# can-lehmann/exprgrad

Hardware: AMD Instinct MI355X
Metric: GFLOP/s matmul 4096^3 f32 (1 GPU) (higher is better)
Workload: dtype f32

## Files before the change

### exprgrad_amd/csrc/kernels/gemm_split_bf16.hip

```cpp
#include <algorithm>
#include <cfloat>

#include "gemm_fused.hpp"
#include "../eg_internal.hpp"
#include "../switches.hpp"

namespace {

typedef __bf16 bf16x8 __attribute__((ext_vector_type(8)));
typedef __bf16 bf16x4 __attribute__((ext_vector_type(4)));
typedef float f32x4 __attribute__((ext_vector_type(4)));


struct SplitOperand {
  const float* src;
  long ld;
  long R;
  int kc;
  __bf16* dst;
};

__device__ __forceinline__ void unit_coords(const SplitOperand& o, long K, long u, long& r, long& chunk) {
  const long cpr = K / 8, t = u >> 6;
  const int l = (int)(u & 63);
  if (o.kc) {
    const long per = cpr / 4;
    r = (t / per) * 16 + (l >> 2);
    chunk = (t % per) * 4 + (l & 3);
  } else {
    const long per = cpr / 2;
    r = (t / per) * 32 + (l >> 1);
    chunk = (t % per) * 2 + (l & 1);
  }
}

__device__ __forceinline__ void load_unit(const SplitOperand& o, long r, long chunk, float (&x)[8]) {
  if (o.kc) {
    const f32x4* p = reinterpret_cast<const f32x4*>(o.src + r * o.ld + chunk * 8);
    const f32x4 v0 = __builtin_nontemporal_load(p), v1 = __builtin_nontemporal_load(p + 1);
#pragma unroll
    for (int j = 0; j < 4; ++j) {
      x[j] = v0[j];
      x[4 + j] = v1[j];
    }
  } else {
    const float* p = o.src + chunk * 8 * o.ld + r;
#pragma unroll
    for (int j = 0; j < 8; ++j) x[j] = __builtin_nontemporal_load(p + j * o.ld);
  }
}

__device__ __forceinline__ void split_elem(float v, __bf16& b0, __bf16& b1, __bf16& b2, bool& bad) {
  b0 = (__bf16)v;
  const float r1 = v - (float)b0;
  b1 = (__bf16)r1;
  const float f1 = (float)b1;
  const float r2 = r1 - f1;
  b2 = (__bf16)r2;
  const float f2 = (float)b2;
  bad |= !(r2 == f2);
  bad |= v != 0.f && __builtin_fabsf(v) < FLT_MIN;
  bad |= (f1 != 0.f && __builtin_fabsf(f1) < FLT_MIN) || (f2 != 0.f && __builtin_fabsf(f2) < FLT_MIN);
}

__device__ __forceinline__ void split_unit(const SplitOperand& o, long K, long r, long chunk, const float (&x)[8], bool& bad) {
  bf16x8 h0, h1, h2;
#pragma unroll
  for (int j = 0; j < 8; ++j) {
    __bf16 b0, b1, b2;
    split_elem(x[j], b0, b1, b2, bad);
    h0[j] = b0;
    h1[j] = b1;
    h2[j] = b2;
  }
  const long plane = o.R * K;
  bf16x8* d = reinterpret_cast<bf16x8*>(o.dst + ((chunk >> 1) * o.R + r) * 16 + (chunk & 1) * 8);
  const long ps = plane / 8;
  d[0] = h0;
  d[ps] = h1;
  d[2 * ps] = h2;
}

constexpr int SPLIT_NT = 256;
constexpr int SPLIT_U = 2;

template <int U>
__device__ __forceinline__ void split_units(const SplitOperand& a, const SplitOperand& b, long K, long units_a, long lo, long hi,
                                            bool& bad) {
  constexpr long STEP = (long)SPLIT_NT * U;
  for (long base = lo; base < hi; base += STEP) {
    float x[U][8];
    long r[U], c[U];
#pragma unroll
    for (int i = 0; i < U; ++i) {
      const long u = base + i * SPLIT_NT + threadIdx.x;
      if (u >= hi) continue;
      const bool in_a = u < units_a;
      unit_coords(in_a ? a : b, K, in_a ? u : u - units_a, r[i], c[i]);
      load_unit(in_a ? a : b, r[i], c[i], x[i]);
    }
#pragma unroll
    for (int i = 0; i < U; ++i) {
      const long u = base + i * SPLIT_NT + threadIdx.x;
      if (u >= hi) continue;
      split_unit(u < units_a ? a : b, K, r[i], c[i], x[i], bad);
    }
  }
}

__global__ __launch_bounds__(SPLIT_NT) void split_planes_kernel(SplitOperand a, SplitOperand b, long K, long units_a, long units,
                                                              unsigned* flag, unsigned epoch) {
  constexpr long STEP = (long)SPLIT_NT * SPLIT_U;
  const long per = ((units + gridDim.x - 1) / gridDim.x + STEP - 1) / STEP * STEP;
  const long lo = (long)blockIdx.x * per, hi = lo + per < units ? lo + per : units;
  bool bad = false;
  split_units<SPLIT_U>(a, b, K, units_a, lo, hi, bad);
  if (__builtin_expect(bad, 0)) *(volatile unsigned*)flag = epoch;
}

constexpr int TILE_R = 256;
constexpr int REC_BYTES = 8 * 32 + 16;
constexpr int IMG_PLANE = (TILE_R / 8) * REC_BYTES;
constexpr int IMG_BYTES = 3 * IMG_PLANE;
constexpr int TILE_BLOCKS_PER_CU = 3;

__device__ __forceinline__ void load_tile(const SplitOperand& o, long kt, long rb, f32x4 (&x)[4]) {
  const int wave = threadIdx.x >> 6, lane = threadIdx.x & 63;
  const float* p = o.src + (kt * 16 + wave * 4) * o.ld + rb * TILE_R + lane * 4;
#pragma unroll
  for (int i = 0; i < 4; ++i) x[i] = __builtin_nontemporal_load(reinterpret_cast<const f32x4*>(p + i * o.ld));
}

__device__ __forceinline__ void split_tile(const f32x4 (&x)[4], unsigned char* img, bool& bad) {
  const int wave = threadIdx.x >> 6, lane = threadIdx.x & 63;
  unsigned char* row = img + (lane >> 1) * REC_BYTES + (lane & 1) * 128 + wave * 8;
#pragma unroll
  for (int c = 0; c < 4; ++c) {
    bf16x4 h0, h1, h2;
#pragma unroll
    for (int i = 0; i < 4; ++i) {
      __bf16 b0, b1, b2;
      split_elem(x[i][c], b0, b1, b2, bad);
      h0[i] = b0;
      h1[i] = b1;
      h2[i] = b2;
    }
    *reinterpret_cast<bf16x4*>(row + c * 32) = h0;
    *reinterpret_cast<bf16x4*>(row + c * 32 + IMG_PLANE) = h1;
    *reinterpret_cast<bf16x4*>(row + c * 32 + 2 * IMG_PLANE) = h2;
  }
}

__device__ __forceinline__ int lane_unit(int lane) {
  const int quad = (lane >> 2) & 7;
  return ((lane >> 5) * 2 + (__builtin_popcount(quad) & 1)) * 16 + (quad >> 1) * 4 + (lane & 3);
}

__device__ __forceinline__ void store_tile(const SplitOperand& o, long K, long kt, long rb, const unsigned char* img) {
  const int wave = threadIdx.x >> 6, lane = threadIdx.x & 63;
  const long plane = o.R * K;
  __bf16* d = o.dst + (kt * o.R + rb * TILE_R) * 16;
#pragma unroll
  for (int p = 0; p < 3; ++p)
#pragma unroll
    for (int i = 0; i < 2; ++i) {
      const int u = (wave * 2 + i) * 64 + lane_unit(lane);
      const bf16x8 v = *reinterpret_cast<const bf16x8*>(img + p * IMG_PLANE + (u >> 4) * REC_BYTES + (u & 15) * 16);
      *reinterpret_cast<bf16x8*>(d + p * plane + u * 8) = v;
    }
}

__global__ __launch_bounds__(SPLIT_NT) void split_tiles_kernel(SplitOperand a, SplitOperand b, long K, int tiled, unsigned* flag,
                                                             unsigned epoch) {
  __shared__ __attribute__((aligned(16))) unsigned char img[2][IMG_BYTES];
  bool bad = false;
  int s = 0;
#pragma unroll
  for (int which = 0; which < 2; ++which) {
    const SplitOperand& o = which ? b : a;
    const long n = o.R * K / (TILE_R * 16);
    const long lo = n * blockIdx.x / gridDim.x, hi = n * (blockIdx.x + 1) / gridDim.x;
    if (!(tiled >> which & 1)) {
      const long units = o.R * K / 8;
      split_units<SPLIT_U>(o, o, K, units, lo * (SPLIT_NT * 2), hi * (SPLIT_NT * 2), bad);
      continue;
    }
    if (lo >= hi) continue;
    const long tr = o.R / TILE_R;
    long kt = lo / tr, rb = lo % tr;
    f32x4 x[4];
    load_tile(o, kt, rb, x);
    for (long t = lo; t < hi; ++t) {
      split_tile(x, img[s], bad);
      long nkt = kt, nrb = rb + 1;
      if (nrb == tr) {
        nrb = 0;
        ++nkt;
      }
      if (t + 1 < hi) load_tile(o, nkt, nrb, x);
      __syncthreads();
      store_tile(o, K, kt, rb, img[s]);
      s ^= 1;
      kt = nkt;
      rb = nrb;
    }
  }
  if (__builtin_expect(bad, 0)) *(volatile unsigned*)flag = epoch;
}


constexpr int BM = 256, BN = 256, WM = 128, WN = 64, NT = 512;
constexpr int STAGES = 3;
constexpr int PLANE_BYTES = BM * 16 * 2;
constexpr int STAGE_BYTES = 6 * PLANE_BYTES;
constexpr int LOADS = STAGE_BYTES / (NT * 16);

struct SplitGemmArgs {
  const __bf16* pa;
  const __bf16* pb;
  float* C;
  const float* bias;
  long M, N, K, ldc;
  int tiles_m, tiles_n;
  int accumulate;
  int skew;
  const unsigned* flag;
  unsigned epoch;
};

__device__ __forceinline__ int xcd_remap(int bid, int nwg) {
  constexpr int NXCD = 8;
  const int q = nwg / NXCD, r = nwg % NXCD;
  const int xcd = bid % NXCD, local = bid / NXCD;
  return (xcd < r ? xcd * (q + 1) : r * (q + 1) + (xcd - r) * q) + local;
}
__device__ __forceinline__ void tile_origin(int wgid, int tiles_m, int tiles_n, long& m_blk, long& n_blk) {
  constexpr int GROUP = 8;
  const int per_group = GROUP * tiles_n;
  const int first_m = (wgid / per_group) * GROUP;
  const int gsize = min(tiles_m - first_m, GROUP);
  const int in_group = wgid % per_group;
  m_blk = (long)(first_m + in_group % gsize) * BM;
  n_blk = (long)(in_group / gsize) * BN;
}

__device__ __forceinline__ const void* uniform_ptr(const void* p) {
  const unsigned long v = reinterpret_cast<unsigned long>(p);
  const unsigned lo = __builtin_amdgcn_readfirstlane((unsigned)v), hi = __builtin_amdgcn_readfirstlane((unsigned)(v >> 32));
  return reinterpret_cast<const void*>(((unsigned long)hi << 32) | lo);
}

constexpr int ROLE_LOAD_OWN = 1, ROLE_LOAD_PARTNER = 2, ROLE_READ_TOP = 4, ROLE_READ_AHEAD = 8;
constexpr int PARTNER = 4;

#ifdef EG_SPLIT_GEMM_STAMPS
constexpr int STAMP_BLOCKS = 1024;
__device__ unsigned long long g_split_stamps[STAMP_BLOCKS][8][4];
#define EG_STAMP(t)                                                                  \
  do {                                                                               \
    __builtin_amdgcn_sched_barrier(0);                                               \
    asm volatile("s_memtime %0\n\ts_waitcnt lgkmcnt(0)" : "=s"(t)::"memory"); \
    __builtin_amdgcn_sched_barrier(0);                                               \
  } while (0)
#else
#define EG_STAMP(t) \
  do {              \
  } while (0)
#endif

__global__ __launch_bounds__(NT) void split_gemm_kernel(SplitGemmArgs a) {
  if (*(volatile const unsigned*)a.flag == a.epoch) return;
  __shared__ __attribute__((aligned(16))) unsigned char lds[STAGES * STAGE_BYTES];

  const int tid = threadIdx.x, lane = tid & 63, wave = __builtin_amdgcn_readfirstlane(tid >> 6);
  const int wr = wave >> 2, wc = wave & 3;
  long m_blk, n_blk;
  tile_origin(xcd_remap(blockIdx.x, gridDim.x), a.tiles_m, a.tiles_n, m_blk, n_blk);

  const __amdgpu_buffer_rsrc_t ra = __builtin_amdgcn_make_buffer_rsrc(
      const_cast<void*>(uniform_ptr(a.pa + m_blk * 16)), (short)0, -1, 0x00020000);
  const __amdgpu_buffer_rsrc_t rb = __builtin_amdgcn_make_buffer_rsrc(
      const_cast<void*>(uniform_ptr(a.pb + n_blk * 16)), (short)0, -1, 0x00020000);
  const unsigned a_plane = (unsigned)(a.M * a.K * 2), b_plane = (unsigned)(a.N * a.K * 2);
  const unsigned a_ktile = (unsigned)(a.M * 32), b_ktile = (unsigned)(a.N * 32);
  const unsigned voff = (unsigned)lane * 16;

  auto pieces = [&](int kt, int s, int w) {
    unsigned char* st = lds + s * STAGE_BYTES + w * 1024;
    const unsigned at = (unsigned)kt * a_ktile + (unsigned)w * 1024, bt = (unsigned)kt * b_ktile + (unsigned)w * 1024;
#pragma unroll
    for (int i = 0; i < LOADS; ++i) {
      __attribute__((address_space(3))) void* dst = (__attribute__((address_space(3))) void*)(st + i * PLANE_BYTES);
      if (i < 3)
        __builtin_amdgcn_raw_ptr_buffer_load_lds(ra, dst, 16, voff, (unsigned)i * a_plane + at, 0, 0);
      else
        __builtin_amdgcn_raw_ptr_buffer_load_lds(rb, dst, 16, voff, (unsigned)(i - 3) * b_plane + bt, 0, 0);
    }
  };
  auto issue = [&](int kt, int s, int r) {
    if (r & ROLE_LOAD_OWN) pieces(kt, s, wave);
    if (r & ROLE_LOAD_PARTNER) pieces(kt, s, wave ^ PARTNER);
  };

  f32x4 acc[8][4];
#pragma unroll
  for (int i = 0; i < 8; ++i)
#pragma unroll
    for (int j = 0; j < 4; ++j)
#pragma unroll
      for (int r = 0; r < 4; ++r) acc[i][j][r] = 0.f;

  const int sel = lane >> 5;
  const int a_row = (wr * WM + (lane & 15)) * 32 + ((lane >> 4) & 1) * 16;
  const int b_row = 3 * PLANE_BYTES + (wc * WN + (lane & 15)) * 32 + ((lane >> 4) & 1) * 16;
  const int a01_off = a_row + sel * PLANE_BYTES, a02_off = a_row + 2 * sel * PLANE_BYTES;
  const int b21_off = b_row + (2 - sel) * PLANE_BYTES, b10_off = b_row + (1 - sel) * PLANE_BYTES, b00_off = b_row;

  bf16x8 fb21[4], fb10[4], fb00[4], fa01, fa02;
  auto read_head = [&](const unsigned char* st) {
#pragma unroll
    for (int j = 0; j < 4; ++j) {
      fb21[j] = *reinterpret_cast<const bf16x8*>(st + b21_off + j * 512);
      fb10[j] = *reinterpret_cast<const bf16x8*>(st + b10_off + j * 512);
      fb00[j] = *reinterpret_cast<const bf16x8*>(st + b00_off + j * 512);
    }
    fa01 = *reinterpret_cast<const bf16x8*>(st + a01_off);
    fa02 = *reinterpret_cast<const bf16x8*>(st + a02_off);
  };
#pragma unroll
  for (int j = 0; j < 4; ++j) fb21[j] = fb10[j] = fb00[j] = bf16x8{};
  fa01 = fa02 = bf16x8{};

  const int skew = a.skew;
  const int role = !skew ? ROLE_LOAD_OWN | ROLE_READ_TOP
                         : (wave & PARTNER) ? ROLE_LOAD_OWN | ROLE_LOAD_PARTNER | ROLE_READ_TOP : ROLE_READ_AHEAD;
  const int KT = (int)(a.K / 16);
  issue(0, 0, role);
  if (KT > 1) issue(1, 1, role);
  if (skew) {
    if (KT > 1) asm volatile("s_waitcnt vmcnt(12)" ::: "memory");
    else asm volatile("s_waitcnt vmcnt(0)" ::: "memory");
    __builtin_amdgcn_s_barrier();
    asm volatile("" ::: "memory");
    if (role & ROLE_READ_AHEAD) read_head(lds);
  }
#ifdef EG_SPLIT_GEMM_STAMPS
  unsigned long long t0 = 0, t1 = 0, t2 = 0, front = 0, body = 0, back = 0;
#endif
  int s = 0;
  for (int kt = 0; kt < KT; ++kt) {
    if (!skew && kt + 1 < KT) asm volatile("s_waitcnt vmcnt(6)" ::: "memory");
    else asm volatile("s_waitcnt vmcnt(0)" ::: "memory");
    __builtin_amdgcn_s_barrier();
    asm volatile("" ::: "memory");
#ifdef EG_SPLIT_GEMM_STAMPS
    EG_STAMP(t0);
    if (kt) back += t0 - t2;
#endif
    int r = role;
    asm volatile("" : "+s"(r));
    if (kt + 2 < KT) issue(kt + 2, s == 0 ? 2 : s - 1, r);
    const unsigned char* st = lds + s * STAGE_BYTES;
    if (r & ROLE_READ_TOP) read_head(st);
    EG_STAMP(t1);
    bf16x8 c01 = fa01, c02 = fa02;
#pragma unroll
    for (int i = 0; i < 8; ++i) {
      bf16x8 n01 = c01, n02 = c02;
      __builtin_amdgcn_sched_barrier(0);
      if (i + 1 < 8) {
        n01 = *reinterpret_cast<const bf16x8*>(st + a01_off + (i + 1) * 512);
        n02 = *reinterpret_cast<const bf16x8*>(st + a02_off + (i + 1) * 512);
      }
      __builtin_amdgcn_sched_barrier(0);
#pragma unroll
      for (int j = 0; j < 4; ++j) acc[i][j] = __builtin_amdgcn_mfma_f32_16x16x32_bf16(c01, fb21[j], acc[i][j], 0, 0, 0);
#pragma unroll
      for (int j = 0; j < 4; ++j) acc[i][j] = __builtin_amdgcn_mfma_f32_16x16x32_bf16(c01, fb10[j], acc[i][j], 0, 0, 0);
#pragma unroll
      for (int j = 0; j < 4; ++j) acc[i][j] = __builtin_amdgcn_mfma_f32_16x16x32_bf16(c02, fb00[j], acc[i][j], 0, 0, 0);
      c01 = n01;
      c02 = n02;
    }
    EG_STAMP(t2);
#ifdef EG_SPLIT_GEMM_STAMPS
    front += t1 - t0;
    body += t2 - t1;
#endif
    s = s == STAGES - 1 ? 0 : s + 1;
    if ((r & ROLE_READ_AHEAD) && kt + 1 < KT) read_head(lds + s * STAGE_BYTES);
  }
#ifdef EG_SPLIT_GEMM_STAMPS
  if (lane == 0 && blockIdx.x < STAMP_BLOCKS) {
    unsigned long long* o = g_split_stamps[blockIdx.x][wave];
    o[0] = front;
    o[1] = body;
    o[2] = back;
    o[3] = (unsigned long long)KT;
  }
#endif

  __syncthreads();
  float* park = reinterpret_cast<float*>(lds) + wave * 64 * WN;
  const int prow = lane >> 4, pc4 = (lane & 15) * 4;
  const long col = n_blk + wc * WN + pc4;
  f32x4 b4 = {0.f, 0.f, 0.f, 0.f};
  if (a.bias) b4 = *reinterpret_cast<const f32x4*>(a.bias + col);
#pragma unroll
  for (int h = 0; h < 2; ++h) {
#pragma unroll
    for (int i = 0; i < 4; ++i)
#pragma unroll
      for (int j = 0; j < 4; ++j)
#pragma unroll
        for (int r = 0; r < 4; ++r) park[(i * 16 + 4 * prow + r) * WN + j * 16 + (lane & 15)] = acc[4 * h + i][j][r];
    asm volatile("s_waitcnt lgkmcnt(0)" ::: "memory");
#pragma unroll
    for (int q = 0; q < 16; ++q) {
      const int row = 4 * q + prow;
      f32x4 v = *reinterpret_cast<const f32x4*>(park + row * WN + pc4);
      f32x4* c = reinterpret_cast<f32x4*>(a.C + (m_blk + wr * WM + h * 64 + row) * a.ldc + col);
      if (a.accumulate) v = *c + v;
      if (a.bias) v = v + b4;
      *c = v;
    }
    asm volatile("s_waitcnt lgkmcnt(0)" ::: "memory");
  }
}

inline bool aligned16(const void* p) { return (reinterpret_cast<uintptr_t>(p) & 15) == 0; }

constexpr size_t kPlaneCap = 1ull << 30;

}

namespace eg {
namespace gemm {

int sgemm_split(eg_ctx* ctx, int trans_a, int trans_b, long M, long N, long K, const float* A, long lda, const float* B, long ldb,
                float* C, long ldc, int accumulate, const float* bias) {
  if (!ctx || !A || !B || !C || M <= 0 || N <= 0 || K <= 0) return EG_ERR_UNSUPPORTED;
  if (lda < (trans_a ? M : K) || ldb < (trans_b ? K : N) || ldc < N) return EG_ERR_UNSUPPORTED;
  if (eg::sw::on(eg::Sw::NO_SPLIT_GEMM)) return EG_ERR_UNSUPPORTED;
  if (M % BM != 0 || N % BN != 0 || K % 32 != 0 || K < 2048) return EG_ERR_UNSUPPORTED;
  if ((M / BM) * (N / BN) < ctx->compute_units) return EG_ERR_UNSUPPORTED;
  const size_t plane_bytes = 6 * (size_t)(M + N) * (size_t)K;
  if (plane_bytes > kPlaneCap || 6 * (size_t)std::max(M, N) * (size_t)K >= (1ull << 31)) return EG_ERR_UNSUPPORTED;
  if (!aligned16(A) || !aligned16(B) || (!trans_a && lda % 4 != 0) || (trans_b && ldb % 4 != 0)) return EG_ERR_UNSUPPORTED;
  if (!aligned16(C) || ldc % 4 != 0 || (bias && !aligned16(bias))) return EG_ERR_UNSUPPORTED;
  if (!exact_single_launch(ctx, trans_a, trans_b, M, N, K, A, lda, B, ldb, C, ldc, bias)) return EG_ERR_UNSUPPORTED;

  int rc = eg::set_device(ctx);
  if (rc) return rc;
  if (!ctx->split_flag) {
    EG_HIP_CHECK(hipMalloc((void**)&ctx->split_flag, sizeof(unsigned)));
    EG_HIP_CHECK(hipMemset(ctx->split_flag, 0, sizeof(unsigned)));
  }
  rc = eg::ensure_workspace(ctx, plane_bytes);
  if (rc) return rc;
  if (++ctx->split_epoch == 0) ctx->split_epoch = 1;
  const unsigned epoch = ctx->split_epoch;

  __bf16* pa = static_cast<__bf16*>(ctx->workspace);
  __bf16* pb = pa + 3 * (size_t)M * K;
  const SplitOperand oa = {A, lda, M, trans_a ? 0 : 1, pa};
  const SplitOperand ob = {B, ldb, N, trans_b ? 1 : 0, pb};
  const bool scalar = eg::sw::on(eg::Sw::SPLIT_PASS_SCALAR);
  const int tiled = (!scalar && !oa.kc && lda % 4 == 0 ? 1 : 0) | (!scalar && !ob.kc && ldb % 4 == 0 ? 2 : 0);
  if (tiled) {
    const long blocks = (long)TILE_BLOCKS_PER_CU * ctx->compute_units;
    hipLaunchKernelGGL(split_tiles_kernel, dim3((unsigned)blocks), dim3(SPLIT_NT), 0, ctx->stream, oa, ob, K, tiled, ctx->split_flag,
                       epoch);
  } else {
    const long units_a = M * K / 8, units = (M + N) * K / 8;
    long blocks = (units + SPLIT_NT * SPLIT_U - 1) / (SPLIT_NT * SPLIT_U);
    if (blocks > 8L * ctx->compute_units) blocks = 8L * ctx->compute_units;
    hipLaunchKernelGGL(split_planes_kernel, dim3((unsigned)blocks), dim3(SPLIT_NT), 0, ctx->stream, oa, ob, K, units_a, units,
                       ctx->split_flag, epoch);
  }
  EG_HIP_CHECK(hipGetLastError());

  SplitGemmArgs g = {};
  g.pa = pa;
  g.pb = pb;
  g.C = C;
  g.bias = bias;
  g.M = M;
  g.N = N;
  g.K = K;
  g.ldc = ldc;
  g.tiles_m = (int)(M / BM);
  g.tiles_n = (int)(N / BN);
  g.accumulate = accumulate;
  g.skew = eg::sw::on(eg::Sw::GEMM_NO_SKEW) ? 0 : 1;
  g.flag = ctx->split_flag;
  g.epoch = epoch;
  hipLaunchKernelGGL(split_gemm_kernel, dim3((unsigned)(g.tiles_m * g.tiles_n)), dim3(NT), 0, ctx->stream, g);
  EG_HIP_CHECK(hipGetLastError());

  return sgemm_exact(ctx, trans_a, trans_b, M, N, K, A, lda, B, ldb, C, ldc, accumulate, bias, ctx->split_flag, epoch);
}

}
}

#ifdef EG_SPLIT_GEMM_STAMPS
extern "C" int eg_debug_split_stamps(unsigned long long* dst, size_t count) {
  if (count > sizeof(g_split_stamps) / sizeof(unsigned long long)) return EG_ERR_UNSUPPORTED;
  EG_HIP_CHECK(hipDeviceSynchronize());
  EG_HIP_CHECK(hipMemcpyFromSymbol(dst, HIP_SYMBOL(g_split_stamps), count * sizeof(unsigned long long)));
  return 0;
}
#endif
```

Baseline: 261,500.

## Add ping-pong split GEMM kernel with producer/consumer wave roles

Adds a templated split_product with a PINGPONG variant. In it, one half of the waves (role Y) issues all global-to-LDS loads for both halves, and the two halves are staggered by one barrier so that their MFMA phases alternate, with s_setprio raising priority during multiply. The default launch now uses the ping-pong kernel, and the old skewed kernel becomes reachable only via the NO_SKEW switch with skew forced to 0. The aim is better overlap of LDS reads, global loads and MFMA across wave groups. The cost is two barriers per k-tile and a more delicate vmcnt schedule.

```diff
diff --git a/exprgrad_amd/csrc/kernels/gemm_split_bf16.hip b/exprgrad_amd/csrc/kernels/gemm_split_bf16.hip
--- a/exprgrad_amd/csrc/kernels/gemm_split_bf16.hip
+++ b/exprgrad_amd/csrc/kernels/gemm_split_bf16.hip
@@ -2,6 +2,7 @@
 #include <cfloat>
 
 #include "gemm_fused.hpp"
+#include "split_schedule.hpp"
 #include "../eg_internal.hpp"
 #include "../switches.hpp"
 
@@ -268,9 +269,40 @@
   } while (0)
 #endif
 
-__global__ __launch_bounds__(NT) void split_gemm_kernel(SplitGemmArgs a) {
+__device__ __forceinline__ void store_c(const SplitGemmArgs& a, unsigned char (&lds)[STAGES * STAGE_BYTES], const f32x4 (&acc)[8][4], long m_blk,
+                                        long n_blk, int wave, int lane) {
+  const int wr = wave >> 2, wc = wave & 3;
+  __syncthreads();
+  float* park = reinterpret_cast<float*>(lds) + wave * 64 * WN;
+  const int prow = lane >> 4, pc4 = (lane & 15) * 4;
+  const long col = n_blk + wc * WN + pc4;
+  f32x4 b4 = {0.f, 0.f, 0.f, 0.f};
+  if (a.bias) b4 = *reinterpret_cast<const f32x4*>(a.bias + col);
+#pragma unroll
+  for (int h = 0; h < 2; ++h) {
+#pragma unroll
+    for (int i = 0; i < 4; ++i)
+#pragma unroll
+      for (int j = 0; j < 4; ++j)
+#pragma unroll
+        for (int r = 0; r < 4; ++r) park[(i * 16 + 4 * prow + r) * WN + j * 16 + (lane & 15)] = acc[4 * h + i][j][r];
+    asm volatile("s_waitcnt lgkmcnt(0)" ::: "memory");
+#pragma unroll
+    for (int q = 0; q < 16; ++q) {
+      const int row = 4 * q + prow;
+      f32x4 v = *reinterpret_cast<const f32x4*>(park + row * WN + pc4);
+      f32x4* c = reinterpret_cast<f32x4*>(a.C + (m_blk + wr * WM + h * 64 + row) * a.ldc + col);
+      if (a.accumulate) v = *c + v;
+      if (a.bias) v = v + b4;
+      *c = v;
+    }
+    asm volatile("s_waitcnt lgkmcnt(0)" ::: "memory");
+  }
+}
+
+template <bool PINGPONG>
+__device__ __forceinline__ void split_product(const SplitGemmArgs& a, unsigned char (&lds)[STAGES * STAGE_BYTES]) {
   if (*(volatile const unsigned*)a.flag == a.epoch) return;
-  __shared__ __attribute__((aligned(16))) unsigned char lds[STAGES * STAGE_BYTES];
 
   const int tid = threadIdx.x, lane = tid & 63, wave = __builtin_amdgcn_readfirstlane(tid >> 6);
   const int wr = wave >> 2, wc = wave & 3;
@@ -330,6 +362,77 @@
 #pragma unroll
   for (int j = 0; j < 4; ++j) fb21[j] = fb10[j] = fb00[j] = bf16x8{};
   fa01 = fa02 = bf16x8{};
+
+  auto multiply = [&](const unsigned char* st) {
+    bf16x8 c01 = fa01, c02 = fa02;
+#pragma unroll
+    for (int i = 0; i < 8; ++i) {
+      bf16x8 n01 = c01, n02 = c02;
+      __builtin_amdgcn_sched_barrier(0);
+      if (i + 1 < 8) {
+        n01 = *reinterpret_cast<const bf16x8*>(st + a01_off + (i + 1) * 512);
+        n02 = *reinterpret_cast<const bf16x8*>(st + a02_off + (i + 1) * 512);
+      }
+      __builtin_amdgcn_sched_barrier(0);
+#pragma unroll
+      for (int j = 0; j < 4; ++j) acc[i][j] = __builtin_amdgcn_mfma_f32_16x16x32_bf16(c01, fb21[j], acc[i][j], 0, 0, 0);
+#pragma unroll
+      for (int j = 0; j < 4; ++j) acc[i][j] = __builtin_amdgcn_mfma_f32_16x16x32_bf16(c01, fb10[j], acc[i][j], 0, 0, 0);
+#pragma unroll
+      for (int j = 0; j < 4; ++j) acc[i][j] = __builtin_amdgcn_mfma_f32_16x16x32_bf16(c02, fb00[j], acc[i][j], 0, 0, 0);
+      c01 = n01;
+      c02 = n02;
+    }
+  };
+
+  if constexpr (PINGPONG) {
+    namespace ss = eg::split_sched;
+    static_assert(ss::STAGES == STAGES && ss::PIECES == 2 * LOADS && ss::WAVES * 64 == NT, "split_schedule.hpp is this kernel's");
+    auto issue_both = [&](int kt, int s) {
+      pieces(kt, s, wave);
+      pieces(kt, s, wave ^ PARTNER);
+    };
+    const int role = ss::role_of(wave);
+    const int KT = (int)(a.K / 16);
+    if (role == ss::Y) {
+      for (int t = 0; t < ss::prologue_tiles(ss::Y, KT); ++t) issue_both(t, ss::stage_of(t));
+      const int fly = ss::prologue_vmcnt(KT);
+      if (fly == 2 * ss::PIECES) asm volatile("s_waitcnt vmcnt(24)" ::: "memory");
+      else if (fly == ss::PIECES) asm volatile("s_waitcnt vmcnt(12)" ::: "memory");
+      else asm volatile("s_waitcnt vmcnt(0)" ::: "memory");
+    }
+    static_assert(ss::barriers_before_loop(ss::X) == 1 && ss::barriers_before_loop(ss::Y) == 2, "barrier S, then Y's stagger");
+    __builtin_amdgcn_s_barrier();
+    if (role == ss::Y) __builtin_amdgcn_s_barrier();
+    asm volatile("" ::: "memory");
+    int s = 0, s2 = 2;
+    for (int kt = 0; kt < KT; ++kt) {
+      int go = __builtin_amdgcn_readfirstlane(ss::load_issues(role, kt, KT) ? 1 : 0);
+      int fly = __builtin_amdgcn_readfirstlane(ss::load_waits(role) ? ss::load_vmcnt(kt, KT) : -1);
+      asm volatile("" : "+s"(go), "+s"(fly));
+      if (go) issue_both(ss::load_issue_tile(kt), s2);
+      const unsigned char* st = lds + s * STAGE_BYTES;
+      read_head(st);
+      static_assert(ss::load_vmcnt(0, 3) == 12 && ss::load_vmcnt(0, 2) == 0, "the counts written out below");
+      if (fly == 12) asm volatile("s_waitcnt vmcnt(12)" ::: "memory");
+      else if (fly == 0) asm volatile("s_waitcnt vmcnt(0)" ::: "memory");
+      __builtin_amdgcn_s_barrier();
+      asm volatile("" ::: "memory");
+      __builtin_amdgcn_s_setprio(1);
+      multiply(st);
+      __builtin_amdgcn_sched_barrier(0);
+      __builtin_amdgcn_s_setprio(0);
+      asm volatile("s_waitcnt lgkmcnt(0)" ::: "memory");
+      __builtin_amdgcn_s_barrier();
+      asm volatile("" ::: "memory");
+      s = s == STAGES - 1 ? 0 : s + 1;
+      s2 = s2 == STAGES - 1 ? 0 : s2 + 1;
+    }
+    static_assert(ss::barriers_after_loop(ss::X) == 1 && ss::barriers_after_loop(ss::Y) == 0, "X catches up");
+    if (role == ss::X) __builtin_amdgcn_s_barrier();
+    store_c(a, lds, acc, m_blk, n_blk, wave, lane);
+    return;
+  }
 
   const int skew = a.skew;
   const int role = !skew ? ROLE_LOAD_OWN | ROLE_READ_TOP
@@ -363,25 +466,7 @@
     const unsigned char* st = lds + s * STAGE_BYTES;
     if (r & ROLE_READ_TOP) read_head(st);
     EG_STAMP(t1);
-    bf16x8 c01 = fa01, c02 = fa02;
-#pragma unroll
-    for (int i = 0; i < 8; ++i) {
-      bf16x8 n01 = c01, n02 = c02;
-      __builtin_amdgcn_sched_barrier(0);
-      if (i + 1 < 8) {
-        n01 = *reinterpret_cast<const bf16x8*>(st + a01_off + (i + 1) * 512);
-        n02 = *reinterpret_cast<const bf16x8*>(st + a02_off + (i + 1) * 512);
-      }
-      __builtin_amdgcn_sched_barrier(0);
-#pragma unroll
-      for (int j = 0; j < 4; ++j) acc[i][j] = __builtin_amdgcn_mfma_f32_16x16x32_bf16(c01, fb21[j], acc[i][j], 0, 0, 0);
-#pragma unroll
-      for (int j = 0; j < 4; ++j) acc[i][j] = __builtin_amdgcn_mfma_f32_16x16x32_bf16(c01, fb10[j], acc[i][j], 0, 0, 0);
-#pragma unroll
-      for (int j = 0; j < 4; ++j) acc[i][j] = __builtin_amdgcn_mfma_f32_16x16x32_bf16(c02, fb00[j], acc[i][j], 0, 0, 0);
-      c01 = n01;
-      c02 = n02;
-    }
+    multiply(st);
     EG_STAMP(t2);
 #ifdef EG_SPLIT_GEMM_STAMPS
     front += t1 - t0;
@@ -399,33 +484,16 @@
     o[3] = (unsigned long long)KT;
   }
 #endif
-
-  __syncthreads();
-  float* park = reinterpret_cast<float*>(lds) + wave * 64 * WN;
-  const int prow = lane >> 4, pc4 = (lane & 15) * 4;
-  const long col = n_blk + wc * WN + pc4;
-  f32x4 b4 = {0.f, 0.f, 0.f, 0.f};
-  if (a.bias) b4 = *reinterpret_cast<const f32x4*>(a.bias + col);
-#pragma unroll
-  for (int h = 0; h < 2; ++h) {
-#pragma unroll
-    for (int i = 0; i < 4; ++i)
-#pragma unroll
-      for (int j = 0; j < 4; ++j)
-#pragma unroll
-        for (int r = 0; r < 4; ++r) park[(i * 16 + 4 * prow + r) * WN + j * 16 + (lane & 15)] = acc[4 * h + i][j][r];
-    asm volatile("s_waitcnt lgkmcnt(0)" ::: "memory");
-#pragma unroll
-    for (int q = 0; q < 16; ++q) {
-      const int row = 4 * q + prow;
-      f32x4 v = *reinterpret_cast<const f32x4*>(park + row * WN + pc4);
-      f32x4* c = reinterpret_cast<f32x4*>(a.C + (m_blk + wr * WM + h * 64 + row) * a.ldc + col);
-      if (a.accumulate) v = *c + v;
-      if (a.bias) v = v + b4;
-      *c = v;
-    }
-    asm volatile("s_waitcnt lgkmcnt(0)" ::: "memory");
-  }
+  store_c(a, lds, acc, m_blk, n_blk, wave, lane);
+}
+
+__global__ __launch_bounds__(NT) void split_gemm_kernel(SplitGemmArgs a) {
+  __shared__ __attribute__((aligned(16))) unsigned char lds[STAGES * STAGE_BYTES];
+  split_product<false>(a, lds);
+}
+__global__ __launch_bounds__(NT) void split_pingpong_kernel(SplitGemmArgs a) {
+  __shared__ __attribute__((aligned(16))) unsigned char lds[STAGES * STAGE_BYTES];
+  split_product<true>(a, lds);
 }
 
 inline bool aligned16(const void* p) { return (reinterpret_cast<uintptr_t>(p) & 15) == 0; }
@@ -492,10 +560,13 @@
   g.tiles_m = (int)(M / BM);
   g.tiles_n = (int)(N / BN);
   g.accumulate = accumulate;
-  g.skew = eg::sw::on(eg::Sw::GEMM_NO_SKEW) ? 0 : 1;
+  g.skew = 0;
   g.flag = ctx->split_flag;
   g.epoch = epoch;
-  hipLaunchKernelGGL(split_gemm_kernel, dim3((unsigned)(g.tiles_m * g.tiles_n)), dim3(NT), 0, ctx->stream, g);
+  if (eg::sw::on(eg::Sw::GEMM_NO_SKEW))
+    hipLaunchKernelGGL(split_gemm_kernel, dim3((unsigned)(g.tiles_m * g.tiles_n)), dim3(NT), 0, ctx->stream, g);
+  else
+    hipLaunchKernelGGL(split_pingpong_kernel, dim3((unsigned)(g.tiles_m * g.tiles_n)), dim3(NT), 0, ctx->stream, g);
   EG_HIP_CHECK(hipGetLastError());
 
   return sgemm_exact(ctx, trans_a, trans_b, M, N, K, A, lda, B, ldb, C, ldc, accumulate, bias, ctx->split_flag, epoch);
diff --git a/exprgrad_amd/csrc/kernels/split_schedule.hpp b/exprgrad_amd/csrc/kernels/split_schedule.hpp
--- /dev/null
+++ b/exprgrad_amd/csrc/kernels/split_schedule.hpp
@@ -0,0 +1,42 @@
+#pragma once
+
+namespace eg {
+namespace split_sched {
+
+constexpr int STAGES = 3;
+constexpr int WAVES = 8;
+constexpr int PIECES = 12;
+constexpr int X = 0, Y = 1;
+
+constexpr int role_of(int wave) { return (wave >> 2) & 1; }
+constexpr int stage_of(int kt) { return kt % STAGES; }
+
+constexpr int prologue_tiles(int role, int KT) { return role != Y ? 0 : KT < STAGES ? KT : STAGES; }
+constexpr int prologue_vmcnt(int KT) { return (prologue_tiles(Y, KT) - 1) * PIECES; }
+constexpr int barriers_before_loop(int role) { return role == Y ? 2 : 1; }
+constexpr int barriers_after_loop(int role) { return role == X ? 1 : 0; }
+
+constexpr bool load_issues(int role, int kt, int KT) { return role == Y && kt >= 1 && kt + 2 < KT; }
+constexpr int load_issue_tile(int kt) { return kt + 2; }
+constexpr bool load_waits(int role) { return role == Y; }
+constexpr int load_vmcnt(int kt, int KT) { return kt + 2 < KT ? PIECES : 0; }
+
+template <class V>
+constexpr void walk(int role, int KT, V& v) {
+  for (int t = 0; t < prologue_tiles(role, KT); ++t) v.issue(t, stage_of(t));
+  if (prologue_tiles(role, KT)) v.wait(prologue_vmcnt(KT));
+  for (int b = 0; b < barriers_before_loop(role); ++b) v.barrier();
+  for (int kt = 0; kt < KT; ++kt) {
+    if (load_issues(role, kt, KT)) v.issue(load_issue_tile(kt), stage_of(load_issue_tile(kt)));
+    v.read(kt, stage_of(kt));
+    if (load_waits(role)) v.wait(load_vmcnt(kt, KT));
+    v.barrier();
+    v.read(kt, stage_of(kt));
+    v.mfma(kt);
+    v.barrier();
+  }
+  for (int b = 0; b < barriers_after_loop(role); ++b) v.barrier();
+}
+
+}
+}
```

Result: faster. 268,700 (median of 6 runs) (+2.7%).
